# NilanEkanayake/TiTok-Video

Hardware: AMD Instinct MI355X
Metric: video clips/sec encode+decode (whole node) (higher is better)
Workload: dtype bf16

## Files before the change

### include/titok_hip.h

```cpp
#ifndef TITOK_HIP_H
#define TITOK_HIP_H

#include <stdint.h>

#ifdef __cplusplus
extern "C" {
#endif

#define TTV_OK 0
#define TTV_ERR_INVALID 1
#define TTV_ERR_LAUNCH 2
#define TTV_ERR_UNSUPPORTED 3

#define TTV_BF16 0
#define TTV_F32 1

#define TTV_ENCODER 0
#define TTV_DECODER 1

#define TTV_MAX_FSQ 8
#define TTV_MAX_TOKEN 64
#define TTV_MAX_CLIPS_PER_LAUNCH 64

const char* ttv_error_string(void);
// ... 56 lines not shown

int64_t ttv_mlp_pack_bytes(int inner, int next_qkv_rows);
int ttv_mlp_pack(const void* w12_folded, const void* w3, const void* out_proj, const void* next_qkv_folded, int next_qkv_rows, int inner,
                 int width, int dtype, void* mlp_packed, void* stream);
int ttv_mlp_fused(const void* x, int ldx, const void* mlp_packed, int inner, void* y, int ldy, const float* post_gain, float alpha,
                  float eps, int M, int width, int dtype, void* stream);
typedef struct ttv_next_qkv {
  void* qkv; int32_t ld;
  const float* rope_cs;
  int32_t rows;
  int32_t rope_q_end, rope_k_begin, rope_k_end;
} ttv_next_qkv;
int ttv_layer_tail_fused(const void* ao, int ldao, const float* attn_post_gain, float attn_alpha, const void* x, int ldx,
                         const void* mlp_packed, int inner, void* y, int ldy, const float* ffd_post_gain, float ffd_alpha, float eps,
                         int M, int width, int dtype, const ttv_next_qkv* next, void* stream);

int ttv_fill_const_rows(void* x, int dtype, int ld, const int32_t* rows_map, int rows, int width, const float* mask_token,
                        const float* gain, float eps, void* stream);
int ttv_decoder_embed(const void* codes, int token_size, const void* w, const void* bias, const float* mask_token, const float* gain,
                      void* x, int dtype, int ld, const int32_t* rows_map, int rows, int width, float eps, void* stream);

#define TTV_ATTN_GATE 1
#define TTV_ATTN_PAIRED 2
#define TTV_ATTN_QSCALED 4
#define TTV_ATTN_ALLFULL 8
#define TTV_ATTN_PIPE 16
#define TTV_ATTN_SPLIT3 32
#define TTV_ATTN_SPLIT_OUT 64
#define TTV_ATTN_SPLIT_IN 128
int ttv_attention(const void* qkvg, int ld, void* out, int ldo, const int32_t* cu_seqlens, const int32_t* qblocks,
// ... 276 lines not shown
```

### titok_video_amd/_lib.py

```python
from __future__ import annotations

import ctypes as C
import os
import threading

import torch

TTV_BF16, TTV_F32 = 0, 1
TTV_ENCODER, TTV_DECODER = 0, 1
TTV_MAX_FSQ = 8
TTV_MAX_TOKEN = 64
TTV_MAX_CLIPS_PER_LAUNCH = 64

_HERE = os.path.dirname(os.path.abspath(__file__))
LIB_PATH = os.environ.get("TTV_LIB_PATH") or os.path.join(_HERE, "libtitok_hip.so")

i32, i64, f32, vp = C.c_int32, C.c_int64, C.c_float, C.c_void_p


class FsqParams(C.Structure):
    _fields_ = [("n", i32), ("levels", i32 * TTV_MAX_FSQ), ("basis", i32 * TTV_MAX_FSQ),
                ("half_l", f32 * TTV_MAX_FSQ), ("offset", f32 * TTV_MAX_FSQ), ("shift", f32 * TTV_MAX_FSQ),
                ("half_width", f32 * TTV_MAX_FSQ)]

# ... 102 lines not shown
    "ttv_linear_fp8_mx": (C.c_int, [vp, C.c_int, vp, vp, vp, C.c_int, vp, vp, vp, C.c_int, C.c_int, C.c_int, C.c_int, C.c_int, vp, C.c_int, C.c_int,
                                    vp, C.c_int, f32, vp]),
    "ttv_rmsnorm": (C.c_int, [vp, C.c_int, C.c_int, vp, vp, C.c_int, C.c_int, vp, vp, C.c_int, C.c_int, f32, vp]),
    "ttv_rope_apply": (C.c_int, [vp, C.c_int, C.c_int, C.c_int, C.c_int, vp, vp]),
    "ttv_linear": (C.c_int, [vp, C.c_int, vp, C.c_int, vp, vp, vp, C.c_int, C.c_int, C.c_int, C.c_int, C.c_int, vp]),
    "ttv_linear_qkv_rope": (C.c_int, [vp, C.c_int, vp, C.c_int, vp, C.c_int, C.c_int, C.c_int, C.c_int, vp, C.c_int, vp]),
    "ttv_linear_geglu": (C.c_int, [vp, C.c_int, vp, C.c_int, vp, C.c_int, C.c_int, C.c_int, C.c_int, C.c_int, vp]),
    "ttv_linear_residual": (C.c_int, [vp, C.c_int, vp, C.c_int, vp, C.c_int, f32, vp, C.c_int, C.c_int, C.c_int, C.c_int,
                                      C.c_int, C.c_int, vp]),
    "ttv_linear_residual_norm": (C.c_int, [vp, C.c_int, vp, C.c_int, vp, C.c_int, f32, vp, f32, vp, C.c_int, C.c_int, C.c_int,
                                           C.c_int, C.c_int, vp]),
    "ttv_mlp_pack_bytes": (C.c_int64, [C.c_int, C.c_int]),
    "ttv_mlp_pack": (C.c_int, [vp, vp, vp, vp, C.c_int, C.c_int, C.c_int, C.c_int, vp, vp]),
    "ttv_layer_tail_fused": (C.c_int, [vp, C.c_int, vp, f32, vp, C.c_int, vp, C.c_int, vp, C.c_int, vp, f32, f32, C.c_int, C.c_int,
                                       C.c_int, vp, vp]),
    "ttv_mlp_fused": (C.c_int, [vp, C.c_int, vp, C.c_int, vp, C.c_int, vp, f32, f32, C.c_int, C.c_int, C.c_int, vp]),
    "ttv_fill_const_rows": (C.c_int, [vp, C.c_int, C.c_int, vp, C.c_int, C.c_int, vp, vp, f32, vp]),
    "ttv_decoder_embed": (C.c_int, [vp, C.c_int, vp, vp, vp, vp, vp, C.c_int, C.c_int, vp, C.c_int, C.c_int, f32, vp]),
    "ttv_attention": (C.c_int, [vp, C.c_int, vp, C.c_int, vp, vp, C.c_int, C.c_int, C.c_int, C.c_int, C.c_int, C.c_int, vp]),
    "ttv_attention64": (C.c_int, [vp, C.c_int, vp, C.c_int, vp, vp, C.c_int, C.c_int, C.c_int, C.c_int, C.c_int, C.c_int, vp]),
    "ttv_patch_gather": (C.c_int, [C.POINTER(vp), vp, C.c_int, C.c_int, C.c_int, C.c_int, C.c_int, C.c_int, vp, C.c_int,
                                   C.c_int, C.c_int, vp]),
    "ttv_patch_scatter": (C.c_int, [vp, C.c_int, vp, C.c_int, C.c_int, C.c_int, C.c_int, C.c_int, C.c_int, C.POINTER(vp),
                                    C.c_int, C.c_int, vp]),
    "ttv_tower_workspace_bytes": (i64, [C.POINTER(TowerDims), C.POINTER(Batch)]),
    "ttv_encoder_forward": (C.c_int, [C.POINTER(TowerDims), C.POINTER(TowerWeights), C.POINTER(Batch), C.POINTER(vp),
                                      C.POINTER(FsqParams), vp, vp, vp, vp, vp, i64, vp]),
    "ttv_decoder_forward": (C.c_int, [C.POINTER(TowerDims), C.POINTER(TowerWeights), C.POINTER(Batch), vp, C.POINTER(vp),
                                      vp, i64, vp]),
    "ttv_tower_tape_bytes": (i64, [C.POINTER(TowerDims), C.POINTER(Batch)]),
# ... 109 lines not shown
```

### titok_video_amd/csrc/ttv_api.hip

```cpp
#include <stdarg.h>
#include <stdio.h>
#include <stdlib.h>
#include <string.h>

#include "ttv_common.h"
#include "ttv_kernels.h"

static thread_local char g_err[512] = "";

void ttv_set_error(const char* fmt, ...) {
  va_list ap;
  va_start(ap, fmt);
  vsnprintf(g_err, sizeof(g_err), fmt, ap);
  va_end(ap);
}

int g_ttv_prof_class = 0;
thread_local int g_ttv_debug = 0;
long long* g_ttv_stamps = nullptr;
static hipEvent_t* g_prof_start = nullptr;
static hipEvent_t* g_prof_stop = nullptr;
static int g_prof_cap = 0, g_prof_n = 0;

TtvProfScope::TtvProfScope(int cls, hipStream_t stream) : slot(-1), s(stream) {
// ... 135 lines not shown
  const int split3 = (dt == TTV_F32 && w->f32_split3) ? 1 : 0;
  const bool gen_ok = (dt == TTV_BF16 && dm != 256) || split3;
  static const bool s3img_env = !(getenv("TTV_SPLIT3_IMAGES") && getenv("TTV_SPLIT3_IMAGES")[0] == '0');
  const int s3img = (split3 && s3img_env && !(g_ttv_debug & 4096)) ? 1 : 0;
  const int nq = 2 * dm + 2 * g;
  bool qkv_ready = false;
  bool rstd_valid = false;
  bool xq_valid = false;
  static const bool attn_pipe = getenv("TTV_ATTN_PIPE") && getenv("TTV_ATTN_PIPE")[0] == '1';
  static const bool lat_env = !(getenv("TTV_ENC_LATENT_LAST") && getenv("TTV_ENC_LATENT_LAST")[0] == '0');
  const bool lat_last = lat_env && !(g_ttv_debug & 524288) && d->kind == TTV_ENCODER && b->qblocks_latent && b->n_qblocks_latent > 0 &&
                        b->latent_rows && b->sum_tokens > 0 && b->sum_tokens < L;
  static const bool pat_env = !(getenv("TTV_DEC_PATCH_LAST") && getenv("TTV_DEC_PATCH_LAST")[0] == '0');
  const bool pat_last = pat_env && !(g_ttv_debug & 2097152) && d->kind == TTV_DECODER && d->layers >= 2 && b->qblocks_patch &&
                        b->n_qblocks_patch > 0 && !split3 && !b->qblocks_paired;
  bool compacted = false;
  for (int i = 0; i < d->layers; ++i) {
    const ttv_layer_weights& lw = w->layers[i];
    static const bool keel_f32 = getenv("TTV_KEEL_F32SUM") && getenv("TTV_KEEL_F32SUM")[0] == '1';
    if (dt == TTV_BF16 && dm != 256 && dm % 128 == 0 && d->inner % 128 == 0 && !keel_f32 && lw.to_qkv_f8 && lw.to_qkv_mx && lw.w12_f8 && lw.w12_mx &&
        lw.out_proj_f8 && lw.out_proj_mx && lw.w3_f8 && lw.w3_mx &&
        !(lat_last && i == d->layers - 1)) {
      TTV_TRY(run_layer_mx(d, lw, b, ws, i, rstd_valid, xq_valid, attn_pipe, s));
      qkv_ready = false;
      continue;
    }
    xq_valid = false;
    const bool f8_qkv = rows_f8(dt, dm, lw.to_qkv_f8, lw.to_qkv_f8_scale, lw.to_qkv_mx, lw.to_qkv_pn);
    const bool f8_w12 = rows_f8(dt, dm, lw.w12_f8, lw.w12_f8_scale, lw.w12_mx, lw.w12_pn);
    float* const f8_scales = reinterpret_cast<float*>(ws.xn + (((size_t)L * dm + 255) & ~(size_t)255));
// ... 28 lines not shown
                                 (s3img ? (TTV_ATTN_SPLIT_OUT | TTV_ATTN_SPLIT_IN) : 0), dt, s));
    else if (pat_last && i == d->layers - 1 && dt == TTV_BF16 && !attn_pipe)
      TTV_TRY(ttvk_attention(ws.qkv, nq, ws.ao, dm, b->cu_seqlens, b->qblocks_patch, b->n_qblocks_patch, d->q_heads, d->kv_heads, d->head_dim,
                             TTV_ATTN_GATE | (b->qblocks_all_full ? TTV_ATTN_ALLFULL : 0) | (q_scaled ? TTV_ATTN_QSCALED : 0), dt, s));
    else if (q_scaled && b->items64 && b->n_items64 > 0 && d->head_dim == 64)
      TTV_TRY(ttvk_attention64(ws.qkv, nq, ws.ao, dm, b->cu_seqlens, b->items64, b->n_items64, d->q_heads, d->kv_heads,
                               TTV_ATTN_GATE | TTV_ATTN_QSCALED, s));
    else
    TTV_TRY(ttvk_attention(ws.qkv, nq, ws.ao, dm, b->cu_seqlens, b->qblocks, b->n_qblocks, d->q_heads, d->kv_heads, d->head_dim,
                           TTV_ATTN_GATE | (b->qblocks_paired ? TTV_ATTN_PAIRED : 0) | (q_scaled ? TTV_ATTN_QSCALED : 0) |
                               (b->qblocks_all_full ? TTV_ATTN_ALLFULL : 0) | (attn_pipe ? TTV_ATTN_PIPE : 0) | (split3 ? TTV_ATTN_SPLIT3 : 0) |
                               (s3img ? (TTV_ATTN_SPLIT_OUT | TTV_ATTN_SPLIT_IN) : 0), dt, s));
    char* cx = ws.x;
    char* cao = ws.ao;
    int Lc = L;
    if (lat_now) {
      const int64_t rb = (int64_t)dm * esize(dt);
      TTV_TRY(ttvk_copy_rows(ws.x, (int64_t)dm * esize(dt), b->latent_rows, ws.xl, (int64_t)dm * esize(dt), nullptr, b->sum_tokens, dm * (int)esize(dt), s));
      TTV_TRY(ttvk_copy_rows(ws.ao, rb, b->latent_rows, ws.aol, rb, nullptr, b->sum_tokens, (int)rb, s));
      cx = ws.xl; cao = ws.aol; Lc = b->sum_tokens;
      compacted = true;
    }
    static const bool keel_f32sum = getenv("TTV_KEEL_F32SUM") && getenv("TTV_KEEL_F32SUM")[0] == '1';
    static const bool use_fused_mlp = !(getenv("TTV_FUSED_MLP") && getenv("TTV_FUSED_MLP")[0] == '0');
    static const bool use_fused_qkv = getenv("TTV_FUSED_QKV") && getenv("TTV_FUSED_QKV")[0] == '1';
    if (use_fused_mlp && ttvk_mlp_fused_supported(dt, dm, d->inner) && lw.mlp_pack) {
      MlpNextQkv nx = {};
      const bool back = use_fused_qkv && i + 1 < d->layers && lw.mlp_pack_qkv_rows == nq && nq % 64 == 0 && dm % 64 == 0 && g % 64 == 0;
      if (back) { nx.qkv = ws.qkv; nx.ld = nq; nx.rope_cs = b->rope_cs; nx.rows = nq; nx.rope_q_end = dm; nx.rope_k_begin = 2 * dm; nx.rope_k_end = 2 * dm + g; }
      TTV_TRY(ttvk_mlp_fused(cao, dm, i == 0 ? nullptr : lw.attn_post_ln, i == 0 ? 1.f : d->alpha, cx, dm, lw.mlp_pack, d->inner,
                             cx, dm, i == 0 ? nullptr : lw.ffd_post_ln, i == 0 ? 1.f : d->alpha, d->eps, Lc, back ? &nx : nullptr, s));
      qkv_ready = back;
      continue;
    }
    GemmArgs o = {};
    o.dtype = dt; o.split3 = split3; o.x_image = s3img;
    o.x = cao; o.ldx = dm; o.w = lw.out_proj; o.ldw = dm; o.M = Lc; o.N = dm; o.K = dm; o.resid = cx; o.ldr = dm;
    if (i == 0) {
      o.alpha = 1.f; o.y = cx; o.ldy = dm;
      TTV_TRY(ttvk_gemm(EPI_RESID_T, o, s));
    } else if (ttvk_gemm_supports_resid_norm(dt, dm, dm)) {
      o.alpha = d->alpha; o.y = cx; o.ldy = dm; o.norm_gain = lw.attn_post_ln; o.eps = d->eps;
      TTV_TRY(ttvk_gemm(EPI_RESID_NORM, o, s));
    } else {
      const bool want = gen_ok && lw.w12_pn && !f8_w12;
      if (dt == TTV_BF16 && !keel_f32sum) {
// ... 214 lines not shown
int ttv_mlp_pack(const void* w12_folded, const void* w3, const void* out_proj, const void* next_qkv_folded, int next_qkv_rows, int inner,
                 int width, int dtype, void* packed, void* stream) {
  if (!ttvk_mlp_fused_supported(dtype, width, inner)) {
    ttv_set_error("mlp_pack: only bf16, width 256, inner %% 32 == 0");
    return TTV_ERR_UNSUPPORTED;
  }
  return ttvk_mlp_pack(w12_folded, w3, out_proj, next_qkv_folded, next_qkv_rows, inner, packed, (hipStream_t)stream);
}

int ttv_mlp_fused(const void* x, int ldx, const void* mlp_packed, int inner, void* y, int ldy, const float* post_gain, float alpha,
                  float eps, int M, int width, int dtype, void* stream) {
  if (!ttvk_mlp_fused_supported(dtype, width, inner)) {
    ttv_set_error("mlp_fused: only bf16, width 256, inner %% 32 == 0");
    return TTV_ERR_UNSUPPORTED;
  }
  return ttvk_mlp_fused(nullptr, 0, nullptr, 1.f, x, ldx, mlp_packed, inner, y, ldy, post_gain, alpha, eps, M, nullptr, (hipStream_t)stream);
}

int ttv_layer_tail_fused(const void* ao, int ldao, const float* attn_post_gain, float attn_alpha, const void* x, int ldx,
                         const void* mlp_packed, int inner, void* y, int ldy, const float* ffd_post_gain, float ffd_alpha, float eps,
                         int M, int width, int dtype, const ttv_next_qkv* next, void* stream) {
  if (!ttvk_mlp_fused_supported(dtype, width, inner)) {
    ttv_set_error("layer_tail_fused: only bf16, width 256, inner %% 32 == 0");
    return TTV_ERR_UNSUPPORTED;
  }
  TTV_CHECK_ARG(ao, "layer_tail_fused: null attention output");
  MlpNextQkv nx = {};
  if (next) { nx.qkv = next->qkv; nx.ld = next->ld; nx.rope_cs = next->rope_cs; nx.rows = next->rows; nx.rope_q_end = next->rope_q_end;
              nx.rope_k_begin = next->rope_k_begin; nx.rope_k_end = next->rope_k_end; }
  return ttvk_mlp_fused(ao, ldao, attn_post_gain, attn_alpha, x, ldx, mlp_packed, inner, y, ldy, ffd_post_gain, ffd_alpha, eps, M,
                        next ? &nx : nullptr, (hipStream_t)stream);
}

int ttv_fill_const_rows(void* x, int dtype, int ld, const int32_t* rows_map, int rows, int width, const float* mask_token,
                        const float* gain, float eps, void* stream) {
  TTV_CHECK_ARG(rows == 0 || (x && rows_map && mask_token && gain), "fill_const_rows: null buffer");
  return ttvk_fill_const_rows(x, dtype, ld, rows_map, rows, width, mask_token, gain, eps, (hipStream_t)stream);
}

int ttv_decoder_embed(const void* codes, int token_size, const void* w, const void* bias, const float* mask_token, const float* gain,
                      void* x, int dtype, int ld, const int32_t* rows_map, int rows, int width, float eps, void* stream) {
  TTV_CHECK_ARG(rows == 0 || (codes && w && bias && mask_token && gain && x && rows_map), "decoder_embed: null buffer");
  return ttvk_dec_embed(codes, token_size, w, bias, mask_token, gain, x, dtype, ld, rows_map, rows, width, eps, (hipStream_t)stream);
}

int ttv_attention(const void* qkvg, int ld, void* out, int ldo, const int32_t* cu_seqlens, const int32_t* qblocks, int n_qblocks,
// ... 298 lines not shown
```

### titok_video_amd/csrc/ttv_kernels.h

```cpp
#pragma once
#include <hip/hip_runtime.h>
#include <stdint.h>

#include "../../include/titok_hip.h"

int ttvk_rmsnorm(const void* in, int in_dtype, int ld_in, const int* src_rows, void* out, int out_dtype, int ld_out,
                 const int* dst_rows, const float* gain, int rows, int d, float eps, hipStream_t s, float* next_rstd = nullptr,
                 void* mx_q = nullptr, void* mx_s = nullptr,
                 int split_image = 0);
int ttvk_row_rstd(const void* in, int dtype, int ld_in, float* rstd, int rows, int d, float eps, hipStream_t s);
int ttvk_copy_rows(const void* src, int64_t ld_src_bytes, const int* src_rows, void* dst, int64_t ld_dst_bytes, const int* dst_rows, int rows,
                   int row_bytes, hipStream_t s);
int ttvk_fill_const_rows(void* x, int dtype, int ld, const int* rows_map, int rows, int d, const float* mask_token,
                         const float* gain, float eps, hipStream_t s);
int ttvk_dec_embed(const void* codes, int C, const void* w, const void* bias, const float* mask_token, const float* gain,
                   void* x, int dtype, int ld, const int* rows_map, int rows, int d, float eps, hipStream_t s);
int ttvk_fsq_forward(const ttv_fsq_params* p, const void* z, int z_dtype, int rows, void* codes, int codes_dtype, int* indices,
                     float* bounded, hipStream_t s);
int ttvk_fsq_indices_to_codes(const ttv_fsq_params* p, const int* indices, int rows, void* codes, int codes_dtype, hipStream_t s);
int ttvk_enc_tail(const void* x, int dtype, int ld, const int* rows_map, int rows, int d, const float* gain, float eps,
                  const void* w, const void* bias, int C, const ttv_fsq_params* fsq, float* z_out, void* codes, int* indices,
                  float* bounded, hipStream_t s);
int ttvk_patch_copy(bool scatter, void* const* clips, const int* clip_desc, int clip0, int n_clips, int pt, int ph, int pw,
                    int C, void* patches, int ld, int dtype, int max_patches, hipStream_t s);
// ... 79 lines not shown
                      float* best_dist, void* workspace, int64_t workspace_bytes, hipStream_t s);
int ttvk_vq_lookup(const void* cb, int dtype, int ldc, const int* indices, int rows, int C, void* codes, int ldo, hipStream_t s);
int ttvk_vq_lookup_bwd(const void* dcodes, int dtype, int ld, const int* indices, int rows, int C, float* dcb, int ldc, hipStream_t s);

bool ttvk_mlp_fused_supported(int dtype, int width, int inner);
struct MlpNextQkv {
  void* qkv; int ld;
  const float* rope_cs;
  int rows;
  int rope_q_end, rope_k_begin, rope_k_end;
};
int64_t ttvk_mlp_pack_bytes(int inner, int next_qkv_rows);
int ttvk_mlp_pack(const void* w12_folded, const void* w3, const void* wo, const void* next_qkv_folded, int next_qkv_rows, int inner,
                  void* packed, hipStream_t s);
int ttvk_mlp_fused(const void* ao, int ldao, const float* front_gain, float front_alpha, const void* x, int ldx, const void* packed,
                   int inner, void* y, int ldy, const float* post_gain, float alpha, float eps, int M, const MlpNextQkv* nq, hipStream_t s);

int ttvk_l1_loss(void* const* recon, void* const* target, void* const* grad, const int* sizes, int n_clips, int total_clips, int dtype,
                 float* loss, hipStream_t s);
int ttvk_sq_err(void* const* recon, void* const* target, const int* sizes, int n_clips, int dtype, int clamp, double* acc2, hipStream_t s);
int ttvk_rmsnorm_bwd_chain(const void* x, int ldx, const void* dy, int lddy, const float* gain1, float* dgain1, float* dx, int lddx,
                           const void* y, int y_dt, int ldy, const float* gain2, float* dgain2, float out_scale, void* cast_out, int ldc, int rows,
                           int d, float eps, int dt, hipStream_t s);
int ttvk_rmsnorm_bwd(const void* x, int x_dt, int ldx, const int* xr, const void* dy, int dy_dt, int lddy, const int* dyr,
                     const float* gain, void* dx, int dx_dt, int lddx, const int* dxr, int acc, float* dgain, int rows, int d, float eps,
                     hipStream_t s);
int ttvk_colsum(const void* a, int dt, int lda, const int* rows_map, int rows, int n, float* out, hipStream_t s);
int ttvk_sumall(const void* a, int dt, int lda, const int* rows_map, int rows, int n, const float* colw, float scale, float* out, hipStream_t s);
int ttvk_gate_fwd(const void* a, int lda, const void* gate, int ldg, void* ag, int ldo, int rows, int d, int dt, hipStream_t s);
int ttvk_gate_bwd(const void* dag, int ldd, const void* a, int lda, const void* gate, int ldg, void* da, int ldda, void* dgate, int lddg,
                  int rows, int d, int dt, float* delta, hipStream_t s);
// ... 71 lines not shown
```

### titok_video_amd/csrc/ttv_mlp.hip

```cpp
#include "ttv_common.h"
#include "ttv_kernels.h"

#define MLP_W12_CHUNKS 2048
#define MLP_W3_CHUNKS 1024
#define MLP_PANEL_CHUNKS (MLP_W12_CHUNKS + MLP_W3_CHUNKS)
#define MLP_WO_CHUNKS (4 * MLP_W12_CHUNKS)

struct MlpDev {
  const bf16_t* x; int ldx;
  const uint4* pack;
  const bf16_t* ao; int ldao;
  const float* front_gain;
  float front_alpha;
  bf16_t* qkv; int ldq;
  const float* rope_cs;
  int nqp, rope_q_end, rope_k_begin, rope_k_end;
  int I;
  bf16_t* y; int ldy;
  const float* post_gain;
  float alpha, eps;
  int M, n_tiles, debug;
  long long* stamps;
};

__global__ void k_mlp_pack(const bf16_t* __restrict__ w12f, const bf16_t* __restrict__ w3, const bf16_t* __restrict__ wo,
                           const bf16_t* __restrict__ wq, int nq_rows, int I, uint4* __restrict__ out) {
  const int np = I / 32;
  const int nqp = (nq_rows + 63) / 64;
  const int o = blockIdx.x * blockDim.x + threadIdx.x;
  if (o >= np * MLP_PANEL_CHUNKS + MLP_WO_CHUNKS + nqp * MLP_W12_CHUNKS) return;
  if (o >= np * MLP_PANEL_CHUNKS + MLP_WO_CHUNKS) {
    const int c = o - np * MLP_PANEL_CHUNKS - MLP_WO_CHUNKS, qp = c / MLP_W12_CHUNKS, cc = c - qp * MLP_W12_CHUNKS;
    const int r = cc >> 5, cp = cc & 31;
    const int ch = (cp & 16) | ((cp & 15) ^ (r & 15));
    int srow = qp * 64 + r;
    srow = srow < nq_rows ? srow : nq_rows - 1;
// ... 53 lines not shown
                 "s_mov_b32 m0, %0"                                                                                \
                 : "=&s"(keep__)                                                                                   \
                 : "v"(lane16), "v"(lane16 + 8192u), "s"(src_), "s"(dst_)                                          \
                 : "memory", "scc");                                                                               \
  } while (0)
#ifdef MLP_STAMPS
#define MLP_STAMP()                                                                                                \
  do {                                                                                                             \
    if (p.stamps && blockIdx.x == 0 && (wave & 3) == 0 && lane == 0 && n_stamp < 64)                               \
      p.stamps[(wave >> 2) * 64 + n_stamp++] = (long long)__builtin_readcyclecounter();                            \
  } while (0)
#else
#define MLP_STAMP() do { (void)n_stamp; } while (0)
#endif

template <int TPB, int T1, int T2, bool GELU_FIRST, bool KEEL, bool FRONT, bool BACK>
__device__ __forceinline__ void mlp_wave(const MlpDev& p, uint4* l12, uint4* l3, uint4* hb, const float* gl, int tile, int wave, int lane,
                                         int P1F, int P2F, int& n_stamp) {
  constexpr int T1A = T1 > 0 ? T1 : 1, T2A = T2 > 0 ? T2 : 1;
  const int l15 = lane & 15, kq = lane >> 4;
  const int np = p.I / 32;
  const uint32_t lane16 = lane * 16;
  const uint32_t lds_l12 = (uint32_t)(uintptr_t)(__attribute__((address_space(3))) void*)l12;
  const uint32_t lds_l3 = (uint32_t)(uintptr_t)(__attribute__((address_space(3))) void*)l3;
#define GLDS_W12(pn_, buf_)                                                                                        \
  do {                                                                                                             \
    const uint4* src__ = p.pack + ((size_t)(pn_) * MLP_PANEL_CHUNKS + wave * 64);                                  \
    const uint32_t dst__ = lds_l12 + ((buf_) * MLP_W12_CHUNKS + wave * 64) * 16;                                   \
    MLP_GLDS_4(src__, dst__);                                                                                      \
  } while (0)
#define GLDS_W3(pn_, buf_)                                                                                         \
  do {                                                                                                             \
    const uint4* src__ = p.pack + ((size_t)(pn_) * MLP_PANEL_CHUNKS + MLP_W12_CHUNKS + wave * 64);                 \
    const uint32_t dst__ = lds_l3 + ((buf_) * MLP_W3_CHUNKS + wave * 64) * 16;                                     \
    MLP_GLDS_2(src__, dst__);                                                                                      \
  } while (0)

  const int tok0 = tile * (16 * TPB) + l15;
  typedef __attribute__((address_space(1))) char gchar;
  typedef __attribute__((address_space(1))) const char gcchar;
  gcchar* const gx = (gcchar*)p.x;
  gcchar* const gao = (gcchar*)p.ao;
  gchar* const gy = (gchar*)p.y;

  MLP_STAMP();
  __syncthreads();

  bf16x8 bfr[T1A][8];
  float rstd[T1A];
  if (FRONT) {
#define GLDS_WO(wp_, buf_)                                                                                         \
  do {                                                                                                             \
    const uint4* src__ = p.pack + ((size_t)np * MLP_PANEL_CHUNKS + (wp_) * MLP_W12_CHUNKS + wave * 64);            \
    const uint32_t dst__ = lds_l12 + ((buf_) * MLP_W12_CHUNKS + wave * 64) * 16;                                   \
    MLP_GLDS_4(src__, dst__);                                                                                      \
  } while (0)
    GLDS_WO(0, 0);
    bf16x8 abf[T1A][8];
#pragma unroll
    for (int j = 0; j < T1; ++j) {
      const int t = tok0 + 16 * (P1F + j);
      const int tc = t < p.M ? t : p.M - 1;
      const uint32_t aoff = ((uint32_t)tc * (uint32_t)p.ldao + kq * 8) * 2u;
#pragma unroll
      for (int s8 = 0; s8 < 8; ++s8) abf[j][s8] = *(const __attribute__((address_space(1))) bf16x8*)(gao + aoff + s8 * 64);
    }
    f32x4 facc[16][T1A];
    __builtin_amdgcn_s_waitcnt(0x0F70);
    __syncthreads();
#pragma unroll
    for (int wp = 0; wp < 4; ++wp) {
      if (wp + 1 < 4) GLDS_WO(wp + 1, (wp + 1) & 1);
      const uint4* img = l12 + (wp & 1) * MLP_W12_CHUNKS;
      bf16x8 a[2][4];
      if constexpr (T1 > 0) {
#pragma unroll
      for (int i = 0; i < 4; ++i) a[0][i] = MLP_LD12(img, i, 0);
// ... 10 lines not shown
            facc[4 * wp + i][j] = __builtin_amdgcn_mfma_f32_16x16x32_bf16(a[s8 & 1][i], abf[j][s8],
                                                                           s8 ? facc[4 * wp + i][j] : (f32x4){0.f, 0.f, 0.f, 0.f}, 0, 0, 0);
        if (s8 + 1 < 8) __builtin_amdgcn_sched_group_barrier(0x100, 4, 0);
        __builtin_amdgcn_sched_group_barrier(0x008, 4 * T1A, 0);
        __builtin_amdgcn_sched_barrier(0);
      }
      }
      __builtin_amdgcn_s_waitcnt(0x0F70);
      __syncthreads();
    }
#undef GLDS_WO
    GLDS_W12(0, 0);
#pragma unroll
    for (int j = 0; j < T1; ++j) {
      const int t = tok0 + 16 * (P1F + j);
      const int tc = t < p.M ? t : p.M - 1;
      const uint32_t roff = ((uint32_t)tc * (uint32_t)p.ldx + kq * 4) * 2u;
      float ss = 0.f;
#pragma unroll
      for (int m = 0; m < 16; ++m) {
        facc[m][j] += p.front_alpha * cvt4(*(const __attribute__((address_space(1))) bf16x4*)(gx + roff + m * 32));
#pragma unroll
        for (int e = 0; e < 4; ++e) ss = fmaf(facc[m][j][e], facc[m][j][e], ss);
      }
      float scale = 1.0f;
      if (p.front_gain) {
        ss = quad16_sum(ss);
        scale = 1.0f / sqrtf(ss * (1.0f / 256.0f) + p.eps);
      }
      float ss2 = 0.f;
#pragma unroll
// ... 13 lines not shown
          for (int e = 0; e < 4; ++e) {
            const float r = (float)q[u][e];
            ss2 = fmaf(r, r, ss2);
          }
        }
        bfr[j][s8] = (bf16x8){q[0][0], q[0][1], q[0][2], q[0][3], q[1][0], q[1][1], q[1][2], q[1][3]};
      }
      ss2 = quad16_sum(ss2);
      rstd[j] = 1.0f / sqrtf(ss2 * (1.0f / 256.0f) + p.eps);
    }
  } else {
    GLDS_W12(0, 0);
#pragma unroll
    for (int j = 0; j < T1; ++j) {
      const int t = tok0 + 16 * (P1F + j);
      const int tc = t < p.M ? t : p.M - 1;
      const uint32_t xoff = ((uint32_t)tc * (uint32_t)p.ldx + kq * 4) * 2u;
#pragma unroll
      for (int s8 = 0; s8 < 8; ++s8) {
        const u32x2_t lo = *(const __attribute__((address_space(1))) u32x2_t*)(gx + xoff + s8 * 64);
        const u32x2_t hi = *(const __attribute__((address_space(1))) u32x2_t*)(gx + xoff + (s8 * 64 + 32));
        bfr[j][s8] = __builtin_bit_cast(bf16x8, (u32x4_t){lo.x, lo.y, hi.x, hi.y});
      }
    }
#pragma unroll
    for (int j = 0; j < T1; ++j) {
      float ss = 0.f;
#pragma unroll
      for (int s8 = 0; s8 < 8; ++s8)
#pragma unroll
        for (int e = 0; e < 8; ++e) {
// ... 123 lines not shown
  uint4* const xres = l12;
  if (FRONT) {
#pragma unroll
    for (int j = 0; j < T1; ++j)
#pragma unroll
      for (int s8 = 0; s8 < 8; ++s8) xres[((P1F + j) * 8 + s8) * 64 + lane] = __builtin_bit_cast(uint4, bfr[j][s8]);
    __syncthreads();
  }

  bf16x8 xq[T2A][8];
  float rstdq[T2A];
#pragma unroll
  for (int j = 0; j < T2; ++j) {
    const int t = tok0 + 16 * (P2F + j);
    const bool tv = t < p.M;
    const int tc = tv ? t : p.M - 1;
    const uint32_t roff = ((uint32_t)tc * (uint32_t)p.ldx + kq * 4) * 2u;
    float ss = 0.f;
#pragma unroll
    for (int s8 = 0; s8 < 8; ++s8) {
      f32x4 rv0, rv1;
      if (FRONT) {
        const bf16x8 rb = __builtin_bit_cast(bf16x8, xres[((P2F + j) * 8 + s8) * 64 + lane]);
        rv0 = (f32x4){(float)rb[0], (float)rb[1], (float)rb[2], (float)rb[3]};
        rv1 = (f32x4){(float)rb[4], (float)rb[5], (float)rb[6], (float)rb[7]};
      } else {
        rv0 = cvt4(*(const __attribute__((address_space(1))) bf16x4*)(gx + roff + (2 * s8) * 32));
        rv1 = cvt4(*(const __attribute__((address_space(1))) bf16x4*)(gx + roff + (2 * s8 + 1) * 32));
      }
      out[2 * s8][j] += p.alpha * rv0;
      out[2 * s8 + 1][j] += p.alpha * rv1;
// ... 114 lines not shown
                          v[2] * rc[i][j].y - v[3] * rs[i][j].y, v[2] * rs[i][j].y + v[3] * rc[i][j].y};
            const bf16x4 q = {(bf16_t)v[0], (bf16_t)v[1], (bf16_t)v[2], (bf16_t)v[3]};
            pk[u] = __builtin_bit_cast(uint2, q);
          }
          const uint4 ox = xchg16_pair(pk[0], pk[1]);
          const u32x4_t ov = {ox.x, ox.y, ox.z, ox.w};
          if (qv[j]) *(__attribute__((address_space(1))) u32x4_t*)(qrow + ip * 64) = ov;
        }
      }
    }
#undef GLDS_WQ
    MLP_STAMP();
  }
#undef GLDS_W12
#undef GLDS_W3
}

template <int TILES, bool KEEL, bool FRONT, bool BACK>
__global__ __launch_bounds__(512, 1) void k_mlp256(MlpDev p) {
  extern __shared__ __attribute__((aligned(16))) uint4 smem[];
  uint4* const l12 = smem;
  uint4* const l3 = smem + 2 * MLP_W12_CHUNKS;
  uint4* const hb = l3 + 2 * MLP_W3_CHUNKS;
  float* const gl = reinterpret_cast<float*>(hb + 2 * TILES * 64);
  if (threadIdx.x < 256) {
    gl[threadIdx.x] = p.post_gain ? p.post_gain[threadIdx.x] : 1.0f;
    gl[256 + threadIdx.x] = (FRONT && p.front_gain) ? p.front_gain[threadIdx.x] : 1.0f;
  }
  const int lane = threadIdx.x & 63;
  const int wave = __builtin_amdgcn_readfirstlane(threadIdx.x >> 6);
  int n_stamp = 0;
  const int tile = blockIdx.x;
  if constexpr (TILES == 9) {
    if (wave < 4) mlp_wave<9, 2, 0, false, KEEL, FRONT, BACK>(p, l12, l3, hb, gl, tile, wave, lane, 2 * wave, 0, n_stamp);
    else if (wave < 6) mlp_wave<9, 0, 3, false, KEEL, FRONT, BACK>(p, l12, l3, hb, gl, tile, wave, lane, 0, 3 * (wave - 4), n_stamp);
    else if (wave == 6) mlp_wave<9, 1, 1, false, KEEL, FRONT, BACK>(p, l12, l3, hb, gl, tile, wave, lane, 8, 6, n_stamp);
    else mlp_wave<9, 0, 2, false, KEEL, FRONT, BACK>(p, l12, l3, hb, gl, tile, wave, lane, 0, 7, n_stamp);
  } else {
    constexpr int NT = TILES / 4;
    constexpr int TA = NT - NT / 2;
    const int g0 = (wave & 3) * NT;
    if (wave < 4) mlp_wave<TILES, TA, NT - TA, false, KEEL, FRONT, BACK>(p, l12, l3, hb, gl, tile, wave, lane, g0, g0 + TA, n_stamp);
    else mlp_wave<TILES, NT - TA, TA, false, KEEL, FRONT, BACK>(p, l12, l3, hb, gl, tile, wave, lane, g0 + TA, g0, n_stamp);
  }
}
#undef MLP_LD12
#undef MLP_GLDS_4
#undef MLP_GLDS_2
#undef MLP_STAMP

bool ttvk_mlp_fused_supported(int dtype, int width, int inner) { return dtype == TTV_BF16 && width == 256 && inner % 32 == 0 && inner > 0; }

int64_t ttvk_mlp_pack_bytes(int inner, int next_qkv_rows) {
  if (inner <= 0 || inner % 32 != 0 || next_qkv_rows < 0) return 0;
  return ((int64_t)(inner / 32) * MLP_PANEL_CHUNKS + MLP_WO_CHUNKS + (int64_t)((next_qkv_rows + 63) / 64) * MLP_W12_CHUNKS) * 16;
}

int ttvk_mlp_pack(const void* w12_folded, const void* w3, const void* wo, const void* next_qkv_folded, int next_qkv_rows, int inner,
                  void* packed, hipStream_t s) {
  TTV_CHECK_ARG(w12_folded && w3 && packed, "mlp_pack: null buffer");
  TTV_CHECK_ARG(inner > 0 && inner % 32 == 0, "mlp_pack: inner %% 32");
  TTV_CHECK_ARG((next_qkv_folded != nullptr) == (next_qkv_rows > 0), "mlp_pack: next_qkv weight and row count must come together");
  TTV_CHECK_ARG(((uintptr_t)w12_folded % 16 == 0) && ((uintptr_t)packed % 16 == 0) && ((uintptr_t)wo % 16 == 0) &&
                    ((uintptr_t)next_qkv_folded % 16 == 0), "mlp_pack: 16-byte alignment");
  const int total = inner / 32 * MLP_PANEL_CHUNKS + MLP_WO_CHUNKS + (next_qkv_rows + 63) / 64 * MLP_W12_CHUNKS;
  hipLaunchKernelGGL(k_mlp_pack, dim3(ttv_cdiv(total, 256)), dim3(256), 0, s, (const bf16_t*)w12_folded, (const bf16_t*)w3,
                     (const bf16_t*)wo, (const bf16_t*)next_qkv_folded, next_qkv_rows, inner, (uint4*)packed);
  TTV_CHECK_LAUNCH("mlp_pack");
  return TTV_OK;
}

int ttvk_mlp_fused(const void* ao, int ldao, const float* front_gain, float front_alpha, const void* x, int ldx, const void* packed,
                   int inner, void* y, int ldy, const float* post_gain, float alpha, float eps, int M, const MlpNextQkv* nq, hipStream_t s) {
  if (M == 0) return TTV_OK;
  TTV_CHECK_ARG(x && packed && y, "mlp_fused: null buffer");
  TTV_CHECK_ARG(inner % 32 == 0 && ldx % 8 == 0 && ldy % 8 == 0 && (!ao || ldao % 8 == 0), "mlp_fused: inner %% 32, leading dims %% 8");
  TTV_CHECK_ARG(((uintptr_t)x % 16 == 0) && ((uintptr_t)packed % 16 == 0) && ((uintptr_t)y % 16 == 0) && ((uintptr_t)ao % 16 == 0),
                "mlp_fused: 16-byte alignment");
  MlpDev d;
  d.x = (const bf16_t*)x; d.ldx = ldx; d.pack = (const uint4*)packed; d.I = inner;
  d.ao = (const bf16_t*)ao; d.ldao = ldao; d.front_gain = front_gain; d.front_alpha = front_alpha;
  d.y = (bf16_t*)y; d.ldy = ldy; d.post_gain = post_gain; d.alpha = alpha; d.eps = eps; d.M = M; d.debug = g_ttv_debug; d.stamps = g_ttv_stamps;
  d.qkv = nullptr; d.ldq = 0; d.rope_cs = nullptr; d.nqp = 0; d.rope_q_end = d.rope_k_begin = d.rope_k_end = 0;
  if (nq) {
    TTV_CHECK_ARG(nq->qkv && nq->rope_cs && nq->rows > 0 && nq->rows % 64 == 0 && nq->ld >= nq->rows && nq->ld % 4 == 0 &&
                      (uintptr_t)nq->qkv % 8 == 0, "mlp_fused: bad next-qkv arguments (rows %% 64, ld %% 4, 8-byte aligned)");
    TTV_CHECK_ARG(nq->rope_q_end % 64 == 0 && nq->rope_k_begin % 64 == 0 && nq->rope_k_end % 64 == 0, "mlp_fused: rotary ranges must be whole heads");
    d.qkv = (bf16_t*)nq->qkv; d.ldq = nq->ld; d.rope_cs = nq->rope_cs; d.nqp = nq->rows / 64;
    d.rope_q_end = nq->rope_q_end; d.rope_k_begin = nq->rope_k_begin; d.rope_k_end = nq->rope_k_end;
  }
  const int cus = 256;
  int tiles = 4;
  long best = -1;
  for (int c = 1; c <= 3; ++c) {
    const long cost = (long)ttv_cdiv(ttv_cdiv(M, 64 * c), cus) * (16 + 19 * c);
    if (best < 0 || cost < best) { best = cost; tiles = 4 * c; }
  }
  if (!nq && !(g_ttv_debug & 32)) {
    const long cost9 = (long)ttv_cdiv(ttv_cdiv(M, 144), cus) * (16 + 14 * 3);
    if (cost9 < best) { best = cost9; tiles = 9; }
  }
  if ((g_ttv_debug & 512) && !nq) tiles = 9;
  if (g_ttv_debug & 8) tiles = 8;
  if (g_ttv_debug & 64) tiles = 4;
  d.n_tiles = ttv_cdiv(M, 16 * tiles);
  const int grid = d.n_tiles;
  const size_t smem = (size_t)(2 * MLP_W12_CHUNKS + 2 * MLP_W3_CHUNKS + 2 * tiles * 64) * sizeof(uint4) + 2048;
  TtvProfScope prof(TTV_KC_GEMM_GEGLU, s);
#define LAUNCH_MLP(TILES_, KEEL_, FRONT_, BACK_)                                                                    \
  do {                                                                                                              \
    (void)hipFuncSetAttribute((const void*)k_mlp256<TILES_, KEEL_, FRONT_, BACK_>, hipFuncAttributeMaxDynamicSharedMemorySize, (int)smem); \
    hipLaunchKernelGGL((k_mlp256<TILES_, KEEL_, FRONT_, BACK_>), dim3(grid), dim3(512), smem, s, d);                \
  } while (0)
#define LAUNCH_MLP_F(TILES_, KEEL_)                                                                                 \
  do {                                                                                                              \
    if (ao && nq) LAUNCH_MLP(TILES_, KEEL_, true, true);                                                            \
    else if (ao) LAUNCH_MLP(TILES_, KEEL_, true, false);                                                            \
    else LAUNCH_MLP(TILES_, KEEL_, false, false);                                                                   \
  } while (0)
#define LAUNCH_MLP_9(KEEL_)                                                                                         \
  do {                                                                                                              \
    if (ao) LAUNCH_MLP(9, KEEL_, true, false);                                                                      \
    else LAUNCH_MLP(9, KEEL_, false, false);                                                                        \
  } while (0)
  TTV_CHECK_ARG(!nq || ao, "mlp_fused: the next-qkv part needs the out_proj front (ttv_layer_tail_fused)");
  if (post_gain) {
    if (tiles == 9) LAUNCH_MLP_9(true); else if (tiles == 12) LAUNCH_MLP_F(12, true); else if (tiles == 8) LAUNCH_MLP_F(8, true); else LAUNCH_MLP_F(4, true);
  } else {
    if (tiles == 9) LAUNCH_MLP_9(false); else if (tiles == 12) LAUNCH_MLP_F(12, false); else if (tiles == 8) LAUNCH_MLP_F(8, false); else LAUNCH_MLP_F(4, false);
  }
#undef LAUNCH_MLP_9
#undef LAUNCH_MLP_F
#undef LAUNCH_MLP
  TTV_CHECK_LAUNCH("mlp_fused");
  return TTV_OK;
}
```

Baseline: 29880.

## Run last encoder layer tail directly on latent rows via row map

In the encoder's latent-only final layer, the fused MLP tail kernel now reads and writes the latent rows in place through a row index map instead of first compacting x and attention output with two copy-rows kernels. It also adds a single-tile (16-token) kernel variant chosen by a cost model when the row count is small, so the few latent rows spread across more CUs. The cost is an extra indirect index load per row and more template instantiations. In-place writes to x assume each mapped row is touched by only one tile.

```diff
diff --git a/include/titok_hip.h b/include/titok_hip.h
--- a/include/titok_hip.h
+++ b/include/titok_hip.h
@@ -94,6 +94,9 @@
 int ttv_layer_tail_fused(const void* ao, int ldao, const float* attn_post_gain, float attn_alpha, const void* x, int ldx,
                          const void* mlp_packed, int inner, void* y, int ldy, const float* ffd_post_gain, float ffd_alpha, float eps,
                          int M, int width, int dtype, const ttv_next_qkv* next, void* stream);
+int ttv_layer_tail_fused_rows(const void* ao, int ldao, const float* attn_post_gain, float attn_alpha, void* x, int ldx,
+                              const void* mlp_packed, int inner, const float* ffd_post_gain, float ffd_alpha, float eps,
+                              const int32_t* rows, int n_rows, int width, int dtype, void* stream);
 
 int ttv_fill_const_rows(void* x, int dtype, int ld, const int32_t* rows_map, int rows, int width, const float* mask_token,
                         const float* gain, float eps, void* stream);
diff --git a/titok_video_amd/_lib.py b/titok_video_amd/_lib.py
--- a/titok_video_amd/_lib.py
+++ b/titok_video_amd/_lib.py
@@ -140,6 +140,7 @@
     "ttv_mlp_pack": (C.c_int, [vp, vp, vp, vp, C.c_int, C.c_int, C.c_int, C.c_int, vp, vp]),
     "ttv_layer_tail_fused": (C.c_int, [vp, C.c_int, vp, f32, vp, C.c_int, vp, C.c_int, vp, C.c_int, vp, f32, f32, C.c_int, C.c_int,
                                        C.c_int, vp, vp]),
+    "ttv_layer_tail_fused_rows": (C.c_int, [vp, C.c_int, vp, f32, vp, C.c_int, vp, C.c_int, vp, f32, f32, vp, C.c_int, C.c_int, C.c_int, vp]),
     "ttv_mlp_fused": (C.c_int, [vp, C.c_int, vp, C.c_int, vp, C.c_int, vp, f32, f32, C.c_int, C.c_int, C.c_int, vp]),
     "ttv_fill_const_rows": (C.c_int, [vp, C.c_int, C.c_int, vp, C.c_int, C.c_int, vp, vp, f32, vp]),
     "ttv_decoder_embed": (C.c_int, [vp, C.c_int, vp, vp, vp, vp, vp, C.c_int, C.c_int, vp, C.c_int, C.c_int, f32, vp]),
diff --git a/titok_video_amd/csrc/ttv_api.hip b/titok_video_amd/csrc/ttv_api.hip
--- a/titok_video_amd/csrc/ttv_api.hip
+++ b/titok_video_amd/csrc/ttv_api.hip
@@ -173,6 +173,8 @@
   static const bool pat_env = !(getenv("TTV_DEC_PATCH_LAST") && getenv("TTV_DEC_PATCH_LAST")[0] == '0');
   const bool pat_last = pat_env && !(g_ttv_debug & 2097152) && d->kind == TTV_DECODER && d->layers >= 2 && b->qblocks_patch &&
                         b->n_qblocks_patch > 0 && !split3 && !b->qblocks_paired;
+  static const bool direct_env = !(getenv("TTV_ENC_LAST_DIRECT") && getenv("TTV_ENC_LAST_DIRECT")[0] == '0');
+  static const bool use_fused_mlp = !(getenv("TTV_FUSED_MLP") && getenv("TTV_FUSED_MLP")[0] == '0');
   bool compacted = false;
   for (int i = 0; i < d->layers; ++i) {
     const ttv_layer_weights& lw = w->layers[i];
@@ -231,7 +233,10 @@
     char* cx = ws.x;
     char* cao = ws.ao;
     int Lc = L;
-    if (lat_now) {
+    const int* row_map = nullptr;
+    if (lat_now && direct_env && dt == TTV_BF16 && dm == 256 && use_fused_mlp && ttvk_mlp_fused_supported(dt, dm, d->inner) && lw.mlp_pack) {
+      row_map = b->latent_rows; Lc = b->sum_tokens;
+    } else if (lat_now) {
       const int64_t rb = (int64_t)dm * esize(dt);
       TTV_TRY(ttvk_copy_rows(ws.x, (int64_t)dm * esize(dt), b->latent_rows, ws.xl, (int64_t)dm * esize(dt), nullptr, b->sum_tokens, dm * (int)esize(dt), s));
       TTV_TRY(ttvk_copy_rows(ws.ao, rb, b->latent_rows, ws.aol, rb, nullptr, b->sum_tokens, (int)rb, s));
@@ -239,14 +244,13 @@
       compacted = true;
     }
     static const bool keel_f32sum = getenv("TTV_KEEL_F32SUM") && getenv("TTV_KEEL_F32SUM")[0] == '1';
-    static const bool use_fused_mlp = !(getenv("TTV_FUSED_MLP") && getenv("TTV_FUSED_MLP")[0] == '0');
     static const bool use_fused_qkv = getenv("TTV_FUSED_QKV") && getenv("TTV_FUSED_QKV")[0] == '1';
     if (use_fused_mlp && ttvk_mlp_fused_supported(dt, dm, d->inner) && lw.mlp_pack) {
       MlpNextQkv nx = {};
-      const bool back = use_fused_qkv && i + 1 < d->layers && lw.mlp_pack_qkv_rows == nq && nq % 64 == 0 && dm % 64 == 0 && g % 64 == 0;
+      const bool back = !row_map && use_fused_qkv && i + 1 < d->layers && lw.mlp_pack_qkv_rows == nq && nq % 64 == 0 && dm % 64 == 0 && g % 64 == 0;
       if (back) { nx.qkv = ws.qkv; nx.ld = nq; nx.rope_cs = b->rope_cs; nx.rows = nq; nx.rope_q_end = dm; nx.rope_k_begin = 2 * dm; nx.rope_k_end = 2 * dm + g; }
       TTV_TRY(ttvk_mlp_fused(cao, dm, i == 0 ? nullptr : lw.attn_post_ln, i == 0 ? 1.f : d->alpha, cx, dm, lw.mlp_pack, d->inner,
-                             cx, dm, i == 0 ? nullptr : lw.ffd_post_ln, i == 0 ? 1.f : d->alpha, d->eps, Lc, back ? &nx : nullptr, s));
+                             cx, dm, i == 0 ? nullptr : lw.ffd_post_ln, i == 0 ? 1.f : d->alpha, d->eps, Lc, back ? &nx : nullptr, row_map, s));
       qkv_ready = back;
       continue;
     }
@@ -491,7 +495,7 @@
     ttv_set_error("mlp_fused: only bf16, width 256, inner %% 32 == 0");
     return TTV_ERR_UNSUPPORTED;
   }
-  return ttvk_mlp_fused(nullptr, 0, nullptr, 1.f, x, ldx, mlp_packed, inner, y, ldy, post_gain, alpha, eps, M, nullptr, (hipStream_t)stream);
+  return ttvk_mlp_fused(nullptr, 0, nullptr, 1.f, x, ldx, mlp_packed, inner, y, ldy, post_gain, alpha, eps, M, nullptr, nullptr, (hipStream_t)stream);
 }
 
 int ttv_layer_tail_fused(const void* ao, int ldao, const float* attn_post_gain, float attn_alpha, const void* x, int ldx,
@@ -506,7 +510,19 @@
   if (next) { nx.qkv = next->qkv; nx.ld = next->ld; nx.rope_cs = next->rope_cs; nx.rows = next->rows; nx.rope_q_end = next->rope_q_end;
               nx.rope_k_begin = next->rope_k_begin; nx.rope_k_end = next->rope_k_end; }
   return ttvk_mlp_fused(ao, ldao, attn_post_gain, attn_alpha, x, ldx, mlp_packed, inner, y, ldy, ffd_post_gain, ffd_alpha, eps, M,
-                        next ? &nx : nullptr, (hipStream_t)stream);
+                        next ? &nx : nullptr, nullptr, (hipStream_t)stream);
+}
+
+int ttv_layer_tail_fused_rows(const void* ao, int ldao, const float* attn_post_gain, float attn_alpha, void* x, int ldx,
+                              const void* mlp_packed, int inner, const float* ffd_post_gain, float ffd_alpha, float eps,
+                              const int32_t* rows, int n_rows, int width, int dtype, void* stream) {
+  if (!ttvk_mlp_fused_supported(dtype, width, inner)) {
+    ttv_set_error("layer_tail_fused_rows: only bf16, width 256, inner %% 32 == 0");
+    return TTV_ERR_UNSUPPORTED;
+  }
+  TTV_CHECK_ARG(ao && (n_rows == 0 || rows), "layer_tail_fused_rows: null attention output or row map");
+  return ttvk_mlp_fused(ao, ldao, attn_post_gain, attn_alpha, x, ldx, mlp_packed, inner, x, ldx, ffd_post_gain, ffd_alpha, eps, n_rows,
+                        nullptr, rows, (hipStream_t)stream);
 }
 
 int ttv_fill_const_rows(void* x, int dtype, int ld, const int32_t* rows_map, int rows, int width, const float* mask_token,
diff --git a/titok_video_amd/csrc/ttv_kernels.h b/titok_video_amd/csrc/ttv_kernels.h
--- a/titok_video_amd/csrc/ttv_kernels.h
+++ b/titok_video_amd/csrc/ttv_kernels.h
@@ -117,7 +117,7 @@
 int ttvk_mlp_pack(const void* w12_folded, const void* w3, const void* wo, const void* next_qkv_folded, int next_qkv_rows, int inner,
                   void* packed, hipStream_t s);
 int ttvk_mlp_fused(const void* ao, int ldao, const float* front_gain, float front_alpha, const void* x, int ldx, const void* packed,
-                   int inner, void* y, int ldy, const float* post_gain, float alpha, float eps, int M, const MlpNextQkv* nq, hipStream_t s);
+                   int inner, void* y, int ldy, const float* post_gain, float alpha, float eps, int M, const MlpNextQkv* nq, const int* rows, hipStream_t s);
 
 int ttvk_l1_loss(void* const* recon, void* const* target, void* const* grad, const int* sizes, int n_clips, int total_clips, int dtype,
                  float* loss, hipStream_t s);
diff --git a/titok_video_amd/csrc/ttv_mlp.hip b/titok_video_amd/csrc/ttv_mlp.hip
--- a/titok_video_amd/csrc/ttv_mlp.hip
+++ b/titok_video_amd/csrc/ttv_mlp.hip
@@ -20,6 +20,7 @@
   const float* post_gain;
   float alpha, eps;
   int M, n_tiles, debug;
+  const int* rows;
   long long* stamps;
 };
 
@@ -103,7 +104,7 @@
 #define MLP_STAMP() do { (void)n_stamp; } while (0)
 #endif
 
-template <int TPB, int T1, int T2, bool GELU_FIRST, bool KEEL, bool FRONT, bool BACK>
+template <int TPB, int T1, int T2, bool GELU_FIRST, bool KEEL, bool FRONT, bool BACK, bool ROWS>
 __device__ __forceinline__ void mlp_wave(const MlpDev& p, uint4* l12, uint4* l3, uint4* hb, const float* gl, int tile, int wave, int lane,
                                          int P1F, int P2F, int& n_stamp) {
   constexpr int T1A = T1 > 0 ? T1 : 1, T2A = T2 > 0 ? T2 : 1;
@@ -126,6 +127,8 @@
   } while (0)
 
   const int tok0 = tile * (16 * TPB) + l15;
+  static_assert(!(ROWS && BACK), "the row map and the fused next-qkv part do not go together (rope_cs / qkv rows are not mapped)");
+#define MLP_ROW(t_) (ROWS ? p.rows[t_] : (t_))
   typedef __attribute__((address_space(1))) char gchar;
   typedef __attribute__((address_space(1))) const char gcchar;
   gcchar* const gx = (gcchar*)p.x;
@@ -149,7 +152,7 @@
 #pragma unroll
     for (int j = 0; j < T1; ++j) {
       const int t = tok0 + 16 * (P1F + j);
-      const int tc = t < p.M ? t : p.M - 1;
+      const int tc = MLP_ROW(t < p.M ? t : p.M - 1);
       const uint32_t aoff = ((uint32_t)tc * (uint32_t)p.ldao + kq * 8) * 2u;
 #pragma unroll
       for (int s8 = 0; s8 < 8; ++s8) abf[j][s8] = *(const __attribute__((address_space(1))) bf16x8*)(gao + aoff + s8 * 64);
@@ -190,7 +193,7 @@
 #pragma unroll
     for (int j = 0; j < T1; ++j) {
       const int t = tok0 + 16 * (P1F + j);
-      const int tc = t < p.M ? t : p.M - 1;
+      const int tc = MLP_ROW(t < p.M ? t : p.M - 1);
       const uint32_t roff = ((uint32_t)tc * (uint32_t)p.ldx + kq * 4) * 2u;
       float ss = 0.f;
 #pragma unroll
@@ -234,7 +237,7 @@
 #pragma unroll
     for (int j = 0; j < T1; ++j) {
       const int t = tok0 + 16 * (P1F + j);
-      const int tc = t < p.M ? t : p.M - 1;
+      const int tc = MLP_ROW(t < p.M ? t : p.M - 1);
       const uint32_t xoff = ((uint32_t)tc * (uint32_t)p.ldx + kq * 4) * 2u;
 #pragma unroll
       for (int s8 = 0; s8 < 8; ++s8) {
@@ -388,7 +391,7 @@
   for (int j = 0; j < T2; ++j) {
     const int t = tok0 + 16 * (P2F + j);
     const bool tv = t < p.M;
-    const int tc = tv ? t : p.M - 1;
+    const int tc = MLP_ROW(tv ? t : p.M - 1);
     const uint32_t roff = ((uint32_t)tc * (uint32_t)p.ldx + kq * 4) * 2u;
     float ss = 0.f;
 #pragma unroll
@@ -533,9 +536,10 @@
   }
 #undef GLDS_W12
 #undef GLDS_W3
+#undef MLP_ROW
 }
 
-template <int TILES, bool KEEL, bool FRONT, bool BACK>
+template <int TILES, bool KEEL, bool FRONT, bool BACK, bool ROWS>
 __global__ __launch_bounds__(512, 1) void k_mlp256(MlpDev p) {
   extern __shared__ __attribute__((aligned(16))) uint4 smem[];
   uint4* const l12 = smem;
@@ -551,16 +555,20 @@
   int n_stamp = 0;
   const int tile = blockIdx.x;
   if constexpr (TILES == 9) {
-    if (wave < 4) mlp_wave<9, 2, 0, false, KEEL, FRONT, BACK>(p, l12, l3, hb, gl, tile, wave, lane, 2 * wave, 0, n_stamp);
-    else if (wave < 6) mlp_wave<9, 0, 3, false, KEEL, FRONT, BACK>(p, l12, l3, hb, gl, tile, wave, lane, 0, 3 * (wave - 4), n_stamp);
-    else if (wave == 6) mlp_wave<9, 1, 1, false, KEEL, FRONT, BACK>(p, l12, l3, hb, gl, tile, wave, lane, 8, 6, n_stamp);
-    else mlp_wave<9, 0, 2, false, KEEL, FRONT, BACK>(p, l12, l3, hb, gl, tile, wave, lane, 0, 7, n_stamp);
+    if (wave < 4) mlp_wave<9, 2, 0, false, KEEL, FRONT, BACK, ROWS>(p, l12, l3, hb, gl, tile, wave, lane, 2 * wave, 0, n_stamp);
+    else if (wave < 6) mlp_wave<9, 0, 3, false, KEEL, FRONT, BACK, ROWS>(p, l12, l3, hb, gl, tile, wave, lane, 0, 3 * (wave - 4), n_stamp);
+    else if (wave == 6) mlp_wave<9, 1, 1, false, KEEL, FRONT, BACK, ROWS>(p, l12, l3, hb, gl, tile, wave, lane, 8, 6, n_stamp);
+    else mlp_wave<9, 0, 2, false, KEEL, FRONT, BACK, ROWS>(p, l12, l3, hb, gl, tile, wave, lane, 0, 7, n_stamp);
+  } else if constexpr (TILES == 1) {
+    if (wave == 0) mlp_wave<1, 1, 0, false, KEEL, FRONT, BACK, ROWS>(p, l12, l3, hb, gl, tile, wave, lane, 0, 0, n_stamp);
+    else if (wave == 5) mlp_wave<1, 0, 1, false, KEEL, FRONT, BACK, ROWS>(p, l12, l3, hb, gl, tile, wave, lane, 0, 0, n_stamp);
+    else mlp_wave<1, 0, 0, false, KEEL, FRONT, BACK, ROWS>(p, l12, l3, hb, gl, tile, wave, lane, 0, 0, n_stamp);
   } else {
     constexpr int NT = TILES / 4;
     constexpr int TA = NT - NT / 2;
     const int g0 = (wave & 3) * NT;
-    if (wave < 4) mlp_wave<TILES, TA, NT - TA, false, KEEL, FRONT, BACK>(p, l12, l3, hb, gl, tile, wave, lane, g0, g0 + TA, n_stamp);
-    else mlp_wave<TILES, NT - TA, TA, false, KEEL, FRONT, BACK>(p, l12, l3, hb, gl, tile, wave, lane, g0 + TA, g0, n_stamp);
+    if (wave < 4) mlp_wave<TILES, TA, NT - TA, false, KEEL, FRONT, BACK, ROWS>(p, l12, l3, hb, gl, tile, wave, lane, g0, g0 + TA, n_stamp);
+    else mlp_wave<TILES, NT - TA, TA, false, KEEL, FRONT, BACK, ROWS>(p, l12, l3, hb, gl, tile, wave, lane, g0 + TA, g0, n_stamp);
   }
 }
 #undef MLP_LD12
@@ -590,13 +598,15 @@
 }
 
 int ttvk_mlp_fused(const void* ao, int ldao, const float* front_gain, float front_alpha, const void* x, int ldx, const void* packed,
-                   int inner, void* y, int ldy, const float* post_gain, float alpha, float eps, int M, const MlpNextQkv* nq, hipStream_t s) {
+                   int inner, void* y, int ldy, const float* post_gain, float alpha, float eps, int M, const MlpNextQkv* nq, const int* rows, hipStream_t s) {
   if (M == 0) return TTV_OK;
   TTV_CHECK_ARG(x && packed && y, "mlp_fused: null buffer");
   TTV_CHECK_ARG(inner % 32 == 0 && ldx % 8 == 0 && ldy % 8 == 0 && (!ao || ldao % 8 == 0), "mlp_fused: inner %% 32, leading dims %% 8");
   TTV_CHECK_ARG(((uintptr_t)x % 16 == 0) && ((uintptr_t)packed % 16 == 0) && ((uintptr_t)y % 16 == 0) && ((uintptr_t)ao % 16 == 0),
                 "mlp_fused: 16-byte alignment");
+  TTV_CHECK_ARG(!rows || (ao && !nq), "mlp_fused: the row map goes with the out_proj front and without the next-qkv part");
   MlpDev d;
+  d.rows = rows;
   d.x = (const bf16_t*)x; d.ldx = ldx; d.pack = (const uint4*)packed; d.I = inner;
   d.ao = (const bf16_t*)ao; d.ldao = ldao; d.front_gain = front_gain; d.front_alpha = front_alpha;
   d.y = (bf16_t*)y; d.ldy = ldy; d.post_gain = post_gain; d.alpha = alpha; d.eps = eps; d.M = M; d.debug = g_ttv_debug; d.stamps = g_ttv_stamps;
@@ -619,35 +629,50 @@
     const long cost9 = (long)ttv_cdiv(ttv_cdiv(M, 144), cus) * (16 + 14 * 3);
     if (cost9 < best) { best = cost9; tiles = 9; }
   }
+  if (ao && !nq) {
+    const long cost1 = (long)ttv_cdiv(ttv_cdiv(M, 16), cus) * 30;
+    if (cost1 < best) { best = cost1; tiles = 1; }
+  }
   if ((g_ttv_debug & 512) && !nq) tiles = 9;
   if (g_ttv_debug & 8) tiles = 8;
   if (g_ttv_debug & 64) tiles = 4;
+  if ((g_ttv_debug & 4194304) && ao && !nq) tiles = 1;
   d.n_tiles = ttv_cdiv(M, 16 * tiles);
   const int grid = d.n_tiles;
   const size_t smem = (size_t)(2 * MLP_W12_CHUNKS + 2 * MLP_W3_CHUNKS + 2 * tiles * 64) * sizeof(uint4) + 2048;
   TtvProfScope prof(TTV_KC_GEMM_GEGLU, s);
-#define LAUNCH_MLP(TILES_, KEEL_, FRONT_, BACK_)                                                                    \
+#define LAUNCH_MLP(TILES_, KEEL_, FRONT_, BACK_, ROWS_)                                                             \
   do {                                                                                                              \
-    (void)hipFuncSetAttribute((const void*)k_mlp256<TILES_, KEEL_, FRONT_, BACK_>, hipFuncAttributeMaxDynamicSharedMemorySize, (int)smem); \
-    hipLaunchKernelGGL((k_mlp256<TILES_, KEEL_, FRONT_, BACK_>), dim3(grid), dim3(512), smem, s, d);                \
+    (void)hipFuncSetAttribute((const void*)k_mlp256<TILES_, KEEL_, FRONT_, BACK_, ROWS_>, hipFuncAttributeMaxDynamicSharedMemorySize, (int)smem); \
+    hipLaunchKernelGGL((k_mlp256<TILES_, KEEL_, FRONT_, BACK_, ROWS_>), dim3(grid), dim3(512), smem, s, d);         \
   } while (0)
 #define LAUNCH_MLP_F(TILES_, KEEL_)                                                                                 \
   do {                                                                                                              \
-    if (ao && nq) LAUNCH_MLP(TILES_, KEEL_, true, true);                                                            \
-    else if (ao) LAUNCH_MLP(TILES_, KEEL_, true, false);                                                            \
-    else LAUNCH_MLP(TILES_, KEEL_, false, false);                                                                   \
+    if (rows) LAUNCH_MLP(TILES_, KEEL_, true, false, true);                                                         \
+    else if (ao && nq) LAUNCH_MLP(TILES_, KEEL_, true, true, false);                                                \
+    else if (ao) LAUNCH_MLP(TILES_, KEEL_, true, false, false);                                                     \
+    else LAUNCH_MLP(TILES_, KEEL_, false, false, false);                                                            \
   } while (0)
 #define LAUNCH_MLP_9(KEEL_)                                                                                         \
   do {                                                                                                              \
-    if (ao) LAUNCH_MLP(9, KEEL_, true, false);                                                                      \
-    else LAUNCH_MLP(9, KEEL_, false, false);                                                                        \
+    if (rows) LAUNCH_MLP(9, KEEL_, true, false, true);                                                              \
+    else if (ao) LAUNCH_MLP(9, KEEL_, true, false, false);                                                          \
+    else LAUNCH_MLP(9, KEEL_, false, false, false);                                                                 \
+  } while (0)
+#define LAUNCH_MLP_S(TILES_, KEEL_)                                                                                 \
+  do {                                                                                                              \
+    if (rows) LAUNCH_MLP(TILES_, KEEL_, true, false, true);                                                         \
+    else LAUNCH_MLP(TILES_, KEEL_, true, false, false);                                                             \
   } while (0)
   TTV_CHECK_ARG(!nq || ao, "mlp_fused: the next-qkv part needs the out_proj front (ttv_layer_tail_fused)");
   if (post_gain) {
+    if (tiles == 1) LAUNCH_MLP_S(1, true); else
     if (tiles == 9) LAUNCH_MLP_9(true); else if (tiles == 12) LAUNCH_MLP_F(12, true); else if (tiles == 8) LAUNCH_MLP_F(8, true); else LAUNCH_MLP_F(4, true);
   } else {
+    if (tiles == 1) LAUNCH_MLP_S(1, false); else
     if (tiles == 9) LAUNCH_MLP_9(false); else if (tiles == 12) LAUNCH_MLP_F(12, false); else if (tiles == 8) LAUNCH_MLP_F(8, false); else LAUNCH_MLP_F(4, false);
   }
+#undef LAUNCH_MLP_S
 #undef LAUNCH_MLP_9
 #undef LAUNCH_MLP_F
 #undef LAUNCH_MLP
```

Result: no change. 29660 (-0.7%).
